# yhn112/DeDLOC

Measured on AMD Instinct MI355X. Metric: samples/sec (whole node) ALBERT-large MLM pretrain at 1/2/4/8 peers, higher is better.
Workload: dtype bf16; 1 GPU; model=albert-large-v2, global_batch=4096, seq_len=512, parallelism=collaborative-dp1, micro_batch=512, grad_accum=1, compression=FLOAT16, optimizer=LAMB, impl=dedloc

## Files before the change

dedloc_amd/csrc/include/dl_attn_tile.h:

```cpp
#pragma once

#include "dl_common.h"

namespace {

typedef __bf16 bf16x8 __attribute__((ext_vector_type(8)));
typedef short s4_t __attribute__((ext_vector_type(4)));
typedef short s8_t __attribute__((ext_vector_type(8)));
typedef __attribute__((address_space(3))) s4_t lds_s4;

constexpr int TILE_BYTES = 64 * 128;
constexpr float NEG_BIG = -1.0e30f;

__device__ __forceinline__ int swzf(int x) { return x ^ ((x & 1) << 2); }
__device__ __forceinline__ int chunk_off(int row, int c) { return row * 128 + ((c ^ swzf((row >> 1) & 7)) << 4); }
__device__ __forceinline__ int crow(int i, int hh) { return (i & 3) + 8 * (i >> 2) + 4 * hh; }

__device__ __forceinline__ floatx16 mfma32(bf16x8 a, bf16x8 b, floatx16 c) {
  return __builtin_amdgcn_mfma_f32_32x32x16_bf16(a, b, c, 0, 0, 0);
}

__device__ __forceinline__ bf16x8 lds_row_frag(const uint8_t* tile, int row, int c) {
  return *reinterpret_cast<const bf16x8*>(tile + chunk_off(row, c));
}

__device__ __forceinline__ s4_t lds_tr(const uint8_t* tile, int row0, int col0, int i) {
  const int row = row0 + (i >> 2);
  const int col = col0 + 4 * (i & 3);
  const int off = chunk_off(row, col >> 3) + ((col & 7) << 1);
  return __builtin_amdgcn_ds_read_tr16_b64_v4i16((lds_s4*)(tile + off));
}

__device__ __forceinline__ bf16x8 tr_operand(const uint8_t* tile, int kbase, int hh, int t, int lane) {
  const int col0 = 32 * t + 16 * ((lane >> 4) & 1);
  const s4_t lo = lds_tr(tile, kbase + 4 * hh, col0, lane & 15);
  const s4_t hi = lds_tr(tile, kbase + 8 + 4 * hh, col0, lane & 15);
  const s8_t v = __builtin_shufflevector(lo, hi, 0, 1, 2, 3, 4, 5, 6, 7);
  return __builtin_bit_cast(bf16x8, v);
}

__device__ __forceinline__ bf16x8 pack_acc(const floatx16& x, int s) {
  bf16x8 b;
#pragma unroll
  for (int e = 0; e < 8; ++e) b[e] = (__bf16)x[8 * s + e];
  return b;
}

__device__ __forceinline__ bf16x8 gload8(const bf16_t* p) { return *reinterpret_cast<const bf16x8*>(p); }

typedef __attribute__((address_space(3))) void lds_void;

__device__ __forceinline__ uint32_t lds_u32(const void* p) {
  return __builtin_amdgcn_readfirstlane((uint32_t)(size_t)(const lds_void*)p);
}
__device__ __forceinline__ void dma16(const void* g, uint32_t lds) {
  asm volatile("s_mov_b32 m0, %0\n\tglobal_load_lds_dwordx4 %1, off" ::"s"(lds), "v"(g) : "memory", "m0");
}
__device__ __forceinline__ void dma4(const void* g, uint32_t lds) {
  asm volatile("s_mov_b32 m0, %0\n\tglobal_load_lds_dword %1, off" ::"s"(lds), "v"(g) : "memory", "m0");
}

__device__ __forceinline__ void wait_vm_all() {
  asm volatile("" ::: "memory");
  __builtin_amdgcn_s_waitcnt(0x0F70);
}
template <typename T>
__device__ __forceinline__ void settle(T& v) { asm volatile("" : "+v"(v)); }

template <int NW = 4>
__device__ __forceinline__ void dma_tile(const bf16_t* g, long ld, int row0, uint8_t* tile, int w, int lane) {
#pragma unroll
  for (int j = 0; j < 8 / NW; ++j) {
    const int p = w + NW * j;
    const int row = 8 * p + (lane >> 3);
    const int c = (lane & 7) ^ swzf((row >> 1) & 7);
    dma16(g + (long)(row0 + row) * ld + c * 8, lds_u32(tile + p * 1024));
  }
}

__device__ __forceinline__ void dma_f32x64(const float* g, uint8_t* dst, int lane) {
  dma4(g + lane, lds_u32(dst));
}

template <int N>
__device__ __forceinline__ void wait_cnt(int ahead) {
  if (ahead >= 2) asm volatile("s_waitcnt vmcnt(%0)" ::"n"(2 * N) : "memory");
  else if (ahead == 1) asm volatile("s_waitcnt vmcnt(%0)" ::"n"(N) : "memory");
  else asm volatile("s_waitcnt vmcnt(0)" ::: "memory");
}
template <int PIECES = 4>
__device__ __forceinline__ void wait_stages(int ahead, bool bias) {
  if (bias) wait_cnt<PIECES + 1>(ahead);
  else wait_cnt<PIECES>(ahead);
}

__device__ __forceinline__ void store4(bf16_t* p, float a, float b, float c, float d) {
  uint2 v;
  v.x = (uint32_t)f2bf(a) | ((uint32_t)f2bf(b) << 16);
  v.y = (uint32_t)f2bf(c) | ((uint32_t)f2bf(d) << 16);
  *reinterpret_cast<uint2*>(p) = v;
}

constexpr float RESCALE_THR = 8.f;

struct BlockId {
  int x, h, b;
};
__device__ __forceinline__ BlockId block_id(int xcd) {
  const int gx = gridDim.x, gy = gridDim.y;
  const int n = gx * gy * gridDim.z;
  int p = blockIdx.x + gx * (blockIdx.y + gy * blockIdx.z);
  if (xcd && (n & 7) == 0) p = (p & 7) * (n >> 3) + (p >> 3);
  return BlockId{p % gx, (p / gx) % gy, p / (gx * gy)};
}

__device__ __forceinline__ int kv_end_of(const int* kvinfo, int B, int b, int S, bool& use_len) {
  use_len = false;
  if (kvinfo == nullptr || kvinfo[B] == 0) return S;
  const int len = kvinfo[b];
  if (len <= 0 || len > S) return S;
  use_len = true;
  return len;
}

template <bool VARLEN>
__device__ __forceinline__ int seq_rows(const int* info, int b, int S) {
  if constexpr (VARLEN) return info[b + 1] - info[b];
  else return S;
}
template <bool VARLEN>
__device__ __forceinline__ long seq_base(const int* info, int b, int S) {
  if constexpr (VARLEN) return info[b];
  else return (long)b * S;
}
template <bool VARLEN>
__device__ __forceinline__ int seq_kv_end(const int* info, int B, int b, int S, bool& use_len) {
  if constexpr (VARLEN) {
    use_len = true;
    return info[B + 1 + b];
  } else {
    return kv_end_of(info, B, b, S, use_len);
  }
}
template <bool VARLEN>
__device__ __forceinline__ long seq_stat(int b, int h, int H, int S, int T, long rb) {
  if constexpr (VARLEN) return (long)h * T + rb;
  else return ((long)b * H + h) * S;
}

__device__ __forceinline__ float vmax3(float a, float b, float c) {
  float r;
  asm("v_max3_f32 %0, %1, %2, %3" : "=v"(r) : "v"(a), "v"(b), "v"(c));
  return r;
}

__device__ __forceinline__ float half_max(float x) {
  const auto r = __builtin_amdgcn_permlane32_swap(__float_as_uint(x), __float_as_uint(x), false, false);
  float m;
  asm("v_max_f32 %0, %1, %2" : "=v"(m) : "v"(__uint_as_float(r[0])), "v"(__uint_as_float(r[1])));
  return m;
}
__device__ __forceinline__ float half_sum(float x) {
  const auto r = __builtin_amdgcn_permlane32_swap(__float_as_uint(x), __float_as_uint(x), false, false);
  return __uint_as_float(r[0]) + __uint_as_float(r[1]);
}

}
```

dedloc_amd/csrc/kernels/attention.hip:

```cpp
#include <cstdlib>
#include <type_traits>

#include "dl_attn_tile.h"
#include "dl_common.h"
#include "dl_kernels.h"

namespace {

constexpr int HD = 64;

struct TileRegs { uint4 a, b; };

__device__ __forceinline__ uint4 tile_ld1(const bf16_t* g, long ld, int row0, int rows_valid, int idx) {
  const int row = min(row0 + (idx >> 3), rows_valid - 1);
  return *reinterpret_cast<const uint4*>(g + (long)row * ld + (idx & 7) * 8);
}

__device__ __forceinline__ void tile_load(TileRegs& t, const bf16_t* g, long ld, int row0, int rows_valid) {
  t.a = tile_ld1(g, ld, row0, rows_valid, threadIdx.x);
  t.b = tile_ld1(g, ld, row0, rows_valid, threadIdx.x + 256);
}

__device__ __forceinline__ void tile_store(const TileRegs& t, uint8_t* tile) {
  const int i0 = threadIdx.x, i1 = threadIdx.x + 256;
  *reinterpret_cast<uint4*>(tile + chunk_off(i0 >> 3, i0 & 7)) = t.a;
  *reinterpret_cast<uint4*>(tile + chunk_off(i1 >> 3, i1 & 7)) = t.b;
}

constexpr int NBUF = 2;
constexpr int STAGE = 2 * TILE_BYTES + 512;


struct FwdCtx {
  const bf16_t* Kg;
  const bf16_t* Vg;
  long ld;
  int S, kv_end;
  const float* mb_g;
  float sl2;
  uint8_t* smem;
  float* mbs;
  int w, lane;
  template <int NW = 4>
  __device__ __forceinline__ void issue(int s) const {
    uint8_t* slot = smem + (s % NBUF) * STAGE;
    dma_tile<NW>(Kg, ld, s * 64, slot, w, lane);
    dma_tile<NW>(Vg, ld, s * 64, slot + TILE_BYTES, w, lane);
    if (mb_g) dma_f32x64(mb_g + s * 64, slot + 2 * TILE_BYTES, lane);
  }
};

__device__ __forceinline__ float key_bias(const FwdCtx& c, int key) {
  return c.mb_g ? c.mb_g[key] : (key < c.kv_end ? 0.f : NEG_BIG);
}

template <bool LEAN, bool RING, int QS, int NW>
__device__ __forceinline__ void fwd_tiles(const FwdCtx& c, int kt0, int kt1, int nt, const bf16x8 (&qf)[QS][4],
                                          floatx16 (&o)[QS][2], float (&m)[QS], float (&l)[QS], int r, int hh,
                                          int lane) {
  TileRegs kr, vr;
  float mbr = 0.f;
  for (int kt = kt0; kt < kt1; ++kt) {
    const uint8_t* Ks;
    const float* mb;
    bool more = false;
    if constexpr (RING) {
      wait_stages<16 / NW>(min(nt - 1 - kt, NBUF - 2), c.mb_g != nullptr);
      __syncthreads();
      if (kt + NBUF - 1 < nt) c.template issue<NW>(kt + NBUF - 1);
      Ks = c.smem + (kt % NBUF) * STAGE;
      mb = reinterpret_cast<const float*>(Ks + 2 * TILE_BYTES);
    } else {
      const int cur = kt & 1;
      Ks = c.smem + cur * 2 * TILE_BYTES;
      mb = c.mbs + cur * 64;
      more = kt + 1 < nt;
      if (more) {
        tile_load(kr, c.Kg, c.ld, (kt + 1) * 64, c.S);
        tile_load(vr, c.Vg, c.ld, (kt + 1) * 64, c.S);
        if (threadIdx.x < 64) mbr = key_bias(c, (kt + 1) * 64 + threadIdx.x);
      }
    }
    const uint8_t* Vs = Ks + TILE_BYTES;
    floatx16 s[QS][2];
#pragma unroll
    for (int u = 0; u < QS; ++u)
#pragma unroll
      for (int j = 0; j < 2; ++j)
#pragma unroll
        for (int i = 0; i < 16; ++i) s[u][j][i] = 0.f;
#pragma unroll
    for (int j = 0; j < 2; ++j)
#pragma unroll
      for (int ks = 0; ks < 4; ++ks) {
        const bf16x8 kfr = lds_row_frag(Ks, 32 * j + r, 2 * ks + hh);
#pragma unroll
        for (int u = 0; u < QS; ++u) s[u][j] = mfma32(kfr, qf[u][ks], s[u][j]);
      }
#pragma unroll
    for (int u = 0; u < QS; ++u) {
      if (!LEAN) {
        if (!RING || c.mb_g) {
#pragma unroll
          for (int j = 0; j < 2; ++j)
#pragma unroll
            for (int i = 0; i < 16; ++i) s[u][j][i] = fmaf(s[u][j][i], c.sl2, mb[32 * j + crow(i, hh)]);
        } else {
#pragma unroll
          for (int j = 0; j < 2; ++j)
#pragma unroll
            for (int i = 0; i < 16; ++i)
              s[u][j][i] = fmaf(s[u][j][i], c.sl2, kt * 64 + 32 * j + crow(i, hh) < c.kv_end ? 0.f : NEG_BIG);
        }
      }
      float mc[4];
#pragma unroll
      for (int q4 = 0; q4 < 4; ++q4) {
        const floatx16& sv = s[u][q4 >> 1];
        const int o8 = (q4 & 1) * 8;
        float v = vmax3(sv[o8], sv[o8 + 1], sv[o8 + 2]);
        v = vmax3(v, sv[o8 + 3], sv[o8 + 4]);
        v = vmax3(v, sv[o8 + 5], sv[o8 + 6]);
        mc[q4] = v;
      }
      float mx = vmax3(vmax3(mc[0], mc[1], s[u][0][7]), vmax3(mc[2], mc[3], s[u][0][15]),
                       vmax3(s[u][1][7], s[u][1][15], mc[0]));
      mx = half_max(mx);
      if (LEAN) mx *= c.sl2;
      const bool grow = mx > m[u] + RESCALE_THR;
      if (__ballot(grow) != 0) {
        const float mn = grow ? mx : m[u];
        const float alpha = __builtin_amdgcn_exp2f(m[u] - mn);
        l[u] *= alpha;
        m[u] = mn;
#pragma unroll
        for (int t = 0; t < 2; ++t)
#pragma unroll
          for (int i = 0; i < 16; ++i) o[u][t][i] *= alpha;
      }
      const float nm = -m[u];
      float rsa[8] = {0.f, 0.f, 0.f, 0.f, 0.f, 0.f, 0.f, 0.f};
#pragma unroll
      for (int j = 0; j < 2; ++j)
#pragma unroll
        for (int i = 0; i < 16; ++i) {
          const float pv = __builtin_amdgcn_exp2f(LEAN ? fmaf(s[u][j][i], c.sl2, nm) : s[u][j][i] + nm);
          s[u][j][i] = pv;
          rsa[i & 7] += pv;
        }
      float rs = ((rsa[0] + rsa[1]) + (rsa[2] + rsa[3])) + ((rsa[4] + rsa[5]) + (rsa[6] + rsa[7]));
      l[u] += half_sum(rs);
    }
#pragma unroll
    for (int j = 0; j < 2; ++j)
#pragma unroll
      for (int ss = 0; ss < 2; ++ss) {
        bf16x8 pb[QS];
#pragma unroll
        for (int u = 0; u < QS; ++u) pb[u] = pack_acc(s[u][j], ss);
#pragma unroll
        for (int t = 0; t < 2; ++t) {
          const bf16x8 vfr = tr_operand(Vs, 32 * j + 16 * ss, hh, t, lane);
#pragma unroll
          for (int u = 0; u < QS; ++u) o[u][t] = mfma32(vfr, pb[u], o[u][t]);
        }
      }
    if constexpr (!RING) {
      if (more) {
        uint8_t* Kn = c.smem + ((kt & 1) ^ 1) * 2 * TILE_BYTES;
        tile_store(kr, Kn);
        tile_store(vr, Kn + TILE_BYTES);
        if (threadIdx.x < 64) c.mbs[((kt & 1) ^ 1) * 64 + threadIdx.x] = mbr;
      }
      __syncthreads();
    }
  }
}

template <bool RING, int QS, int NW = 4, bool VARLEN = false>
__global__ __launch_bounds__(64 * NW, NW == 8 ? 1 : 2) void attn_fwd_kernel(const bf16_t* __restrict__ qkv, long ld,
                                                          const float* __restrict__ mbias,
                                                          const int* __restrict__ kvinfo, bf16_t* __restrict__ out,
                                                          long ldo, float* __restrict__ lse, int B, int H, int S_,
                                                          float sl2, int xcd) {
  __shared__ __attribute__((aligned(16))) uint8_t smem[RING ? NBUF * STAGE : 4 * TILE_BYTES + 2 * 64 * 4];
  const BlockId bid = block_id(xcd);
  const int b = bid.b, h = bid.h;
  const int lane = threadIdx.x & 63, w = threadIdx.x >> 6, r = lane & 31, hh = lane >> 5;
  const int S = seq_rows<VARLEN>(kvinfo, b, S_);
  if constexpr (VARLEN) {
    if (bid.x * (32 * QS * NW) >= S) return;
  }
  const long rb = seq_base<VARLEN>(kvinfo, b, S);
  const bf16_t* Qg = qkv + rb * ld + h * HD;
  bool use_len;
  FwdCtx c;
  c.Kg = qkv + rb * ld + (long)H * HD + h * HD;
  c.Vg = qkv + rb * ld + 2L * H * HD + h * HD;
  c.ld = ld;
  c.S = S;
  c.kv_end = seq_kv_end<VARLEN>(kvinfo, B, b, S, use_len);
  c.mb_g = (!use_len && mbias) ? mbias + rb : nullptr;
  c.sl2 = sl2;
  c.smem = smem;
  c.mbs = reinterpret_cast<float*>(smem + 4 * TILE_BYTES);
  c.w = w;
  c.lane = lane;

  static_assert(NW == 4 || (NW == 8 && RING), "8-wave blocks stage through the ring");
  const int nt = (c.kv_end + 63) / 64;
  if constexpr (RING) {
    for (int s0 = 0; s0 < NBUF - 1 && s0 < nt; ++s0) c.template issue<NW>(s0);
  }
  int q[QS];
  bf16x8 qf[QS][4];
#pragma unroll
  for (int u = 0; u < QS; ++u) {
    q[u] = bid.x * (32 * QS * NW) + w * (32 * QS) + 32 * u + r;
    const int qc = min(q[u], S - 1);
#pragma unroll
    for (int ks = 0; ks < 4; ++ks) qf[u][ks] = gload8(Qg + (long)qc * ld + ks * 16 + 8 * hh);
    if constexpr (RING) {
#pragma unroll
      for (int ks = 0; ks < 4; ++ks) settle(qf[u][ks]);
    }
  }

  floatx16 o[QS][2];
  float m[QS], l[QS];
#pragma unroll
  for (int u = 0; u < QS; ++u) {
    m[u] = NEG_BIG;
    l[u] = 0.f;
#pragma unroll
    for (int t = 0; t < 2; ++t)
#pragma unroll
      for (int i = 0; i < 16; ++i) o[u][t][i] = 0.f;
  }

  if constexpr (RING) {
    wait_vm_all();
  } else {
    TileRegs kr, vr;
    tile_load(kr, c.Kg, ld, 0, S);
    tile_load(vr, c.Vg, ld, 0, S);
    const float mbr = threadIdx.x < 64 ? key_bias(c, threadIdx.x) : 0.f;
    tile_store(kr, smem);
    tile_store(vr, smem + TILE_BYTES);
    if (threadIdx.x < 64) c.mbs[threadIdx.x] = mbr;
    __syncthreads();
  }
  const int nlean = c.mb_g ? 0 : c.kv_end / 64;
  fwd_tiles<true, RING, QS, NW>(c, 0, nlean, nt, qf, o, m, l, r, hh, lane);
  fwd_tiles<false, RING, QS, NW>(c, nlean, nt, nt, qf, o, m, l, r, hh, lane);

#pragma unroll
  for (int u = 0; u < QS; ++u) {
    if (q[u] < S) {
      const float inv = 1.f / l[u];
      bf16_t* op = out + (rb + q[u]) * ldo + h * HD;
#pragma unroll
      for (int t = 0; t < 2; ++t)
#pragma unroll
        for (int v = 0; v < 4; ++v)
          store4(op + 32 * t + 8 * v + 4 * hh, o[u][t][4 * v] * inv, o[u][t][4 * v + 1] * inv,
                 o[u][t][4 * v + 2] * inv, o[u][t][4 * v + 3] * inv);
      if (hh == 0) lse[seq_stat<VARLEN>(b, h, H, S, S_, rb) + q[u]] = m[u] + log2f(l[u]);
    }
  }
}

template <bool RING, int QS, bool VARLEN = false>
__global__ __launch_bounds__(256, 2) void attn_bwd_dq_kernel(const bf16_t* __restrict__ qkv, long ld,
                                                             const float* __restrict__ mbias,
                                                             const int* __restrict__ kvinfo,
                                                             const bf16_t* __restrict__ out, const bf16_t* __restrict__ dout,
                                                             long ldo, const float* __restrict__ lse,
                                                             float* __restrict__ delta, bf16_t* __restrict__ dqkv,
                                                             float* __restrict__ dbias, int B, int H, int S_, float sl2,
                                                             float scale, int xcd) {
  __shared__ __attribute__((aligned(16))) uint8_t smem[RING ? NBUF * STAGE : 4 * TILE_BYTES + 4 * 64 * 4];
  const BlockId bid = block_id(xcd);
  const int b = bid.b, h = bid.h;
  const int lane = threadIdx.x & 63, w = threadIdx.x >> 6, r = lane & 31, hh = lane >> 5;
  const int S = seq_rows<VARLEN>(kvinfo, b, S_);
  if constexpr (VARLEN) {
    if (bid.x * (128 * QS) >= S) return;
  }
  const long rb = seq_base<VARLEN>(kvinfo, b, S);
  const bf16_t* Qg = qkv + rb * ld + h * HD;
  const bf16_t* Kg = qkv + rb * ld + (long)H * HD + h * HD;
  const bf16_t* Vg = qkv + rb * ld + 2L * H * HD + h * HD;
  bool use_len;
  const int kv_end = seq_kv_end<VARLEN>(kvinfo, B, b, S, use_len);
  const float* mb_g = (!use_len && mbias) ? mbias + rb : nullptr;
  float* mbs = reinterpret_cast<float*>(smem + 4 * TILE_BYTES);
  const int nt = (kv_end + 63) / 64;
  auto issue = [&](int st) {
    uint8_t* slot = smem + (st % NBUF) * STAGE;
    dma_tile(Kg, ld, st * 64, slot, w, lane);
    dma_tile(Vg, ld, st * 64, slot + TILE_BYTES, w, lane);
    if (mb_g) dma_f32x64(mb_g + st * 64, slot + 2 * TILE_BYTES, lane);
  };
  if constexpr (RING) {
    for (int s0 = 0; s0 < NBUF - 1 && s0 < nt; ++s0) issue(s0);
  }

  int q[QS];
  bf16x8 qf[QS][4], df[QS][4];
  float dl[QS], l2[QS];
#pragma unroll
  for (int u = 0; u < QS; ++u) {
    q[u] = bid.x * (128 * QS) + w * (32 * QS) + 32 * u + r;
    const int qc = min(q[u], S - 1);
    dl[u] = 0.f;
#pragma unroll
    for (int ks = 0; ks < 4; ++ks) {
      qf[u][ks] = gload8(Qg + (long)qc * ld + ks * 16 + 8 * hh);
      const long oo = (rb + qc) * ldo + h * HD + ks * 16 + 8 * hh;
      df[u][ks] = gload8(dout + oo);
      const bf16x8 of = gload8(out + oo);
#pragma unroll
      for (int e = 0; e < 8; ++e) dl[u] += (float)df[u][ks][e] * (float)of[e];
    }
    dl[u] += __shfl_xor(dl[u], 32, 64);
    l2[u] = lse[seq_stat<VARLEN>(b, h, H, S, S_, rb) + qc];
    if constexpr (RING) {
      settle(l2[u]);
      settle(dl[u]);
#pragma unroll
      for (int ks = 0; ks < 4; ++ks) {
        settle(qf[u][ks]);
        settle(df[u][ks]);
      }
    }
  }

  floatx16 dq[QS][2];
#pragma unroll
  for (int u = 0; u < QS; ++u)
#pragma unroll
    for (int t = 0; t < 2; ++t)
#pragma unroll
      for (int i = 0; i < 16; ++i) dq[u][t][i] = 0.f;

  TileRegs kr, vr;
  float mbr = 0.f;
  if constexpr (RING) {
    wait_vm_all();
  } else {
    tile_load(kr, Kg, ld, 0, S);
    tile_load(vr, Vg, ld, 0, S);
    if (threadIdx.x < 64) mbr = mb_g ? mb_g[threadIdx.x] : 0.f;
    tile_store(kr, smem);
    tile_store(vr, smem + TILE_BYTES);
    if (threadIdx.x < 64) mbs[threadIdx.x] = mbr;
    __syncthreads();
  }

  for (int kt = 0; kt < nt; ++kt) {
    const uint8_t* Ks;
    const float* mb;
    if constexpr (RING) {
      wait_stages(min(nt - 1 - kt, NBUF - 2), mb_g != nullptr);
      __syncthreads();
      if (kt + NBUF - 1 < nt) issue(kt + NBUF - 1);
      Ks = smem + (kt % NBUF) * STAGE;
      mb = reinterpret_cast<const float*>(Ks + 2 * TILE_BYTES);
    } else {
      Ks = smem + (kt & 1) * 2 * TILE_BYTES;
      mb = mbs + (kt & 1) * 64;
      if (kt + 1 < nt) {
        tile_load(kr, Kg, ld, (kt + 1) * 64, S);
        tile_load(vr, Vg, ld, (kt + 1) * 64, S);
        if (threadIdx.x < 64) mbr = mb_g ? mb_g[(kt + 1) * 64 + threadIdx.x] : 0.f;
      }
    }
    const uint8_t* Vs = Ks + TILE_BYTES;
    const bool interior = mb_g == nullptr && (kt + 1) * 64 <= kv_end;
#pragma unroll
    for (int j = 0; j < 2; ++j) {
      floatx16 st[QS], dp[QS];
#pragma unroll
      for (int u = 0; u < QS; ++u)
#pragma unroll
        for (int i = 0; i < 16; ++i) { st[u][i] = 0.f; dp[u][i] = 0.f; }
#pragma unroll
      for (int ks = 0; ks < 4; ++ks) {
        const bf16x8 kfr = lds_row_frag(Ks, 32 * j + r, 2 * ks + hh);
        const bf16x8 vfr = lds_row_frag(Vs, 32 * j + r, 2 * ks + hh);
#pragma unroll
        for (int u = 0; u < QS; ++u) {
          st[u] = mfma32(kfr, qf[u][ks], st[u]);
          dp[u] = mfma32(vfr, df[u][ks], dp[u]);
        }
      }
#pragma unroll
      for (int u = 0; u < QS; ++u) {
        if (interior) {
#pragma unroll
          for (int i = 0; i < 16; ++i) {
            const float p = __builtin_amdgcn_exp2f(fmaf(st[u][i], sl2, -l2[u]));
            st[u][i] = p * (dp[u][i] - dl[u]);
          }
        } else {
#pragma unroll
          for (int i = 0; i < 16; ++i) {
            const int key = kt * 64 + 32 * j + crow(i, hh);
            const float bias = mb_g ? mb[32 * j + crow(i, hh)] : (key < kv_end ? 0.f : NEG_BIG);
            const float p = __builtin_amdgcn_exp2f(st[u][i] * sl2 + bias - l2[u]);
            st[u][i] = p * (dp[u][i] - dl[u]);
          }
        }
      }
#pragma unroll
      for (int ss = 0; ss < 2; ++ss) {
        bf16x8 pb[QS];
#pragma unroll
        for (int u = 0; u < QS; ++u) pb[u] = pack_acc(st[u], ss);
#pragma unroll
        for (int t = 0; t < 2; ++t) {
          const bf16x8 ktr = tr_operand(Ks, 32 * j + 16 * ss, hh, t, lane);
#pragma unroll
          for (int u = 0; u < QS; ++u) dq[u][t] = mfma32(ktr, pb[u], dq[u][t]);
        }
      }
    }
    if constexpr (!RING) {
      if (kt + 1 < nt) {
        uint8_t* Kn = smem + ((kt & 1) ^ 1) * 2 * TILE_BYTES;
        tile_store(kr, Kn);
        tile_store(vr, Kn + TILE_BYTES);
        if (threadIdx.x < 64) mbs[((kt & 1) ^ 1) * 64 + threadIdx.x] = mbr;
      }
      __syncthreads();
    }
  }
  if constexpr (RING) __syncthreads();
#pragma unroll
  for (int u = 0; u < QS; ++u) {
    if (q[u] < S && hh == 0) delta[seq_stat<VARLEN>(b, h, H, S, S_, rb) + q[u]] = dl[u];
    if (q[u] < S) {
      bf16_t* dp_ = dqkv + (rb + q[u]) * ld + h * HD;
#pragma unroll
      for (int t = 0; t < 2; ++t)
#pragma unroll
        for (int v = 0; v < 4; ++v)
          store4(dp_ + 32 * t + 8 * v + 4 * hh, dq[u][t][4 * v] * scale, dq[u][t][4 * v + 1] * scale,
                 dq[u][t][4 * v + 2] * scale, dq[u][t][4 * v + 3] * scale);
    }
  }
  if (dbias) {
    float* red = reinterpret_cast<float*>(smem);
    float* part = red + 4 * 32 * 64;
    auto chunk_addr = [&](int row, int ch) { return red + (w * 32 + row) * 64 + ((ch ^ (row & 15)) << 2); };
#pragma unroll
    for (int u = 0; u < QS; ++u) {
      const bool live = q[u] < S;
#pragma unroll
      for (int which = 0; which < 2; ++which) {
        if (which == 0) {
#pragma unroll
          for (int t = 0; t < 2; ++t)
#pragma unroll
            for (int v4 = 0; v4 < 4; ++v4) {
              float4 v = float4{0.f, 0.f, 0.f, 0.f};
              if (live)
                v = float4{round_bf16(dq[u][t][4 * v4] * scale), round_bf16(dq[u][t][4 * v4 + 1] * scale),
                           round_bf16(dq[u][t][4 * v4 + 2] * scale), round_bf16(dq[u][t][4 * v4 + 3] * scale)};
              *reinterpret_cast<float4*>(chunk_addr(r, 8 * t + 2 * v4 + hh)) = v;
            }
        } else {
#pragma unroll
          for (int ks = 0; ks < 4; ++ks)
#pragma unroll
            for (int g = 0; g < 2; ++g) {
              float4 v = float4{0.f, 0.f, 0.f, 0.f};
              if (live)
                v = float4{(float)df[u][ks][4 * g], (float)df[u][ks][4 * g + 1], (float)df[u][ks][4 * g + 2],
                           (float)df[u][ks][4 * g + 3]};
              *reinterpret_cast<float4*>(chunk_addr(r, 4 * ks + 2 * hh + g)) = v;
            }
        }
        __syncthreads();
        {
          const int c = lane;
          float sum = 0.f;
#pragma unroll 8
          for (int row = 0; row < 32; ++row)
            sum += red[(w * 32 + row) * 64 + (((c >> 2) ^ (row & 15)) << 2) + (c & 3)];
          part[w * 64 + c] = sum;
        }
        __syncthreads();
        if (threadIdx.x < 64) {
          const int c = threadIdx.x;
          atomicAdd(&dbias[(which ? 2L * H * HD : 0L) + h * HD + c],
                    part[c] + part[64 + c] + part[128 + c] + part[192 + c]);
        }
        __syncthreads();
      }
    }
  }
}

template <bool RING, int KS, bool VARLEN = false>
__global__ __launch_bounds__(256, KS == 2 ? 1 : 2) void attn_bwd_dkdv_kernel(
    const bf16_t* __restrict__ qkv, long ld, const float* __restrict__ mbias, const int* __restrict__ kvinfo,
    const bf16_t* __restrict__ dout, long ldo, const float* __restrict__ lse, const float* __restrict__ delta,
    bf16_t* __restrict__ dqkv, int B, int H, int S_, float sl2, float scale, int xcd) {
  __shared__ __attribute__((aligned(16))) uint8_t smem[RING ? NBUF * STAGE : 4 * TILE_BYTES + 2 * 2 * 64 * 4];
  const BlockId bid = block_id(xcd);
  const int b = bid.b, h = bid.h;
  const int lane = threadIdx.x & 63, w = threadIdx.x >> 6, r = lane & 31, hh = lane >> 5;
  const int S = seq_rows<VARLEN>(kvinfo, b, S_);
  if constexpr (VARLEN) {
    if (bid.x * (128 * KS) >= S) return;
  }
  const long rb = seq_base<VARLEN>(kvinfo, b, S);
  const bf16_t* Qg = qkv + rb * ld + h * HD;
  const bf16_t* Kg = qkv + rb * ld + (long)H * HD + h * HD;
  const bf16_t* Vg = qkv + rb * ld + 2L * H * HD + h * HD;
  const bf16_t* dOg = dout + rb * ldo + h * HD;
  const float* lse_g = lse + seq_stat<VARLEN>(b, h, H, S, S_, rb);
  const float* del_g = delta + seq_stat<VARLEN>(b, h, H, S, S_, rb);
  float* rowv = reinterpret_cast<float*>(smem + 4 * TILE_BYTES);

  int k[KS];
#pragma unroll
  for (int u = 0; u < KS; ++u) k[u] = bid.x * (128 * KS) + w * (32 * KS) + 32 * u + r;
  bool use_len;
  const int kv_end = seq_kv_end<VARLEN>(kvinfo, B, b, S, use_len);
  if (use_len && bid.x * (128 * KS) >= kv_end) {
#pragma unroll
    for (int u = 0; u < KS; ++u) {
      if (k[u] < S) {
        bf16_t* dkp = dqkv + (rb + k[u]) * ld + (long)H * HD + h * HD;
        bf16_t* dvp = dqkv + (rb + k[u]) * ld + 2L * H * HD + h * HD;
#pragma unroll
        for (int v = 0; v < 8; ++v) {
          store4(dkp + 8 * v + 4 * hh, 0.f, 0.f, 0.f, 0.f);
          store4(dvp + 8 * v + 4 * hh, 0.f, 0.f, 0.f, 0.f);
        }
      }
    }
    return;
  }
  const int nt = S / 64;
  auto issue = [&](int st) {
    uint8_t* slot = smem + (st % NBUF) * STAGE;
    dma_tile(Qg, ld, st * 64, slot, w, lane);
    dma_tile(dOg, ldo, st * 64, slot + TILE_BYTES, w, lane);
    dma_f32x64((w < 2 ? lse_g : del_g) + st * 64, slot + 2 * TILE_BYTES + (w < 2 ? 0 : 256), lane);
  };
  if constexpr (RING) {
    for (int s0 = 0; s0 < NBUF - 1 && s0 < nt; ++s0) issue(s0);
  }
  bf16x8 kf[KS][4], vf[KS][4];
  float mbk[KS];
#pragma unroll
  for (int u = 0; u < KS; ++u) {
    const int kc = min(k[u], S - 1);
#pragma unroll
    for (int ks = 0; ks < 4; ++ks) {
      kf[u][ks] = gload8(Kg + (long)kc * ld + ks * 16 + 8 * hh);
      vf[u][ks] = gload8(Vg + (long)kc * ld + ks * 16 + 8 * hh);
    }
    mbk[u] = use_len ? (k[u] < kv_end ? 0.f : NEG_BIG) : (mbias ? mbias[rb + kc] : 0.f);
    if constexpr (RING) {
      settle(mbk[u]);
#pragma unroll
      for (int ks = 0; ks < 4; ++ks) {
        settle(kf[u][ks]);
        settle(vf[u][ks]);
      }
    }
  }

  floatx16 dk[KS][2], dv[KS][2];
#pragma unroll
  for (int u = 0; u < KS; ++u)
#pragma unroll
    for (int t = 0; t < 2; ++t)
#pragma unroll
      for (int i = 0; i < 16; ++i) { dk[u][t][i] = 0.f; dv[u][t][i] = 0.f; }

  TileRegs qr, dr;
  float rv = 0.f;
  if constexpr (RING) {
    wait_vm_all();
  } else {
    tile_load(qr, Qg, ld, 0, S);
    tile_load(dr, dOg, ldo, 0, S);
    if (threadIdx.x < 128) rv = threadIdx.x < 64 ? lse_g[threadIdx.x] : del_g[threadIdx.x - 64];
    tile_store(qr, smem);
    tile_store(dr, smem + TILE_BYTES);
    if (threadIdx.x < 128) rowv[threadIdx.x] = rv;
    __syncthreads();
  }

  auto qloop = [&](auto lean_tag) {
  constexpr bool LEAN = decltype(lean_tag)::value;
  for (int qt = 0; qt < nt; ++qt) {
    const uint8_t* Qs;
    const float* lse_s;
    if constexpr (RING) {
      wait_stages(min(nt - 1 - qt, NBUF - 2), true);
      __syncthreads();
      if (qt + NBUF - 1 < nt) issue(qt + NBUF - 1);
      Qs = smem + (qt % NBUF) * STAGE;
      lse_s = reinterpret_cast<const float*>(Qs + 2 * TILE_BYTES);
    } else {
      Qs = smem + (qt & 1) * 2 * TILE_BYTES;
      lse_s = rowv + (qt & 1) * 128;
      if (qt + 1 < nt) {
        tile_load(qr, Qg, ld, (qt + 1) * 64, S);
        tile_load(dr, dOg, ldo, (qt + 1) * 64, S);
        if (threadIdx.x < 128)
          rv = threadIdx.x < 64 ? lse_g[(qt + 1) * 64 + threadIdx.x] : del_g[(qt + 1) * 64 + threadIdx.x - 64];
      }
    }
    const uint8_t* Ds = Qs + TILE_BYTES;
    const float* del_s = lse_s + 64;
#pragma unroll
    for (int i2 = 0; i2 < 2; ++i2) {
      floatx16 sc[KS], dp[KS];
#pragma unroll
      for (int u = 0; u < KS; ++u)
#pragma unroll
        for (int i = 0; i < 16; ++i) { sc[u][i] = 0.f; dp[u][i] = 0.f; }
#pragma unroll
      for (int ks = 0; ks < 4; ++ks) {
        const bf16x8 qfr = lds_row_frag(Qs, 32 * i2 + r, 2 * ks + hh);
        const bf16x8 dfr = lds_row_frag(Ds, 32 * i2 + r, 2 * ks + hh);
#pragma unroll
        for (int u = 0; u < KS; ++u) {
          sc[u] = mfma32(qfr, kf[u][ks], sc[u]);
          dp[u] = mfma32(dfr, vf[u][ks], dp[u]);
        }
      }
#pragma unroll
      for (int u = 0; u < KS; ++u)
#pragma unroll
        for (int i = 0; i < 16; ++i) {
          const int qq = 32 * i2 + crow(i, hh);
          const float p = __builtin_amdgcn_exp2f(LEAN ? fmaf(sc[u][i], sl2, -lse_s[qq])
                                                      : sc[u][i] * sl2 + mbk[u] - lse_s[qq]);
          sc[u][i] = p;
          dp[u][i] = p * (dp[u][i] - del_s[qq]);
        }
#pragma unroll
      for (int ss = 0; ss < 2; ++ss) {
        bf16x8 pb[KS], db[KS];
#pragma unroll
        for (int u = 0; u < KS; ++u) {
          pb[u] = pack_acc(sc[u], ss);
          db[u] = pack_acc(dp[u], ss);
        }
#pragma unroll
        for (int t = 0; t < 2; ++t) {
          const bf16x8 dtr = tr_operand(Ds, 32 * i2 + 16 * ss, hh, t, lane);
          const bf16x8 qtr = tr_operand(Qs, 32 * i2 + 16 * ss, hh, t, lane);
#pragma unroll
          for (int u = 0; u < KS; ++u) {
            dv[u][t] = mfma32(dtr, pb[u], dv[u][t]);
            dk[u][t] = mfma32(qtr, db[u], dk[u][t]);
          }
        }
      }
    }
    if constexpr (!RING) {
      if (qt + 1 < nt) {
        uint8_t* Qn = smem + ((qt & 1) ^ 1) * 2 * TILE_BYTES;
        tile_store(qr, Qn);
        tile_store(dr, Qn + TILE_BYTES);
        if (threadIdx.x < 128) rowv[((qt & 1) ^ 1) * 128 + threadIdx.x] = rv;
      }
      __syncthreads();
    }
  }
  };
  if (use_len) {
    qloop(std::true_type{});
#pragma unroll
    for (int u = 0; u < KS; ++u)
      if (k[u] >= kv_end)
#pragma unroll
        for (int t = 0; t < 2; ++t)
#pragma unroll
          for (int i = 0; i < 16; ++i) dk[u][t][i] = dv[u][t][i] = 0.f;
  } else {
    qloop(std::false_type{});
  }
#pragma unroll
  for (int u = 0; u < KS; ++u) {
    if (k[u] < S) {
      bf16_t* dkp = dqkv + (rb + k[u]) * ld + (long)H * HD + h * HD;
      bf16_t* dvp = dqkv + (rb + k[u]) * ld + 2L * H * HD + h * HD;
#pragma unroll
      for (int t = 0; t < 2; ++t)
#pragma unroll
        for (int v = 0; v < 4; ++v) {
          store4(dkp + 32 * t + 8 * v + 4 * hh, dk[u][t][4 * v] * scale, dk[u][t][4 * v + 1] * scale,
                 dk[u][t][4 * v + 2] * scale, dk[u][t][4 * v + 3] * scale);
          store4(dvp + 32 * t + 8 * v + 4 * hh, dv[u][t][4 * v], dv[u][t][4 * v + 1], dv[u][t][4 * v + 2],
                 dv[u][t][4 * v + 3]);
        }
    }
  }
}

constexpr int kAttnXcd = 1;

}

int dl_attn_fwd(const bf16_t* qkv, long ld, const float* mbias, const int* kvinfo, bf16_t* out, long ldo, float* lse,
                int B, int H, int S, int D, float scale, hipStream_t st) {
  if (D == 128) return dl_attn_hd128_fwd(qkv, ld, mbias, kvinfo, out, ldo, lse, B, H, S, scale, st);
  if (D != HD || S % 64 != 0 || ld % 8 != 0 || ldo % 8 != 0) return -1;
  const float sl2 = scale * 1.4426950408889634f;
  dim3 grid((S + 255) / 256, H, B);
  attn_fwd_kernel<true, 2><<<grid, 256, 0, st>>>(qkv, ld, mbias, kvinfo, out, ldo, lse, B, H, S, sl2, kAttnXcd);
  return 0;
}

int dl_attn_bwd(const bf16_t* qkv, long ld, const float* mbias, const int* kvinfo, const bf16_t* out,
                const bf16_t* dout, long ldo, const float* lse, float* delta, bf16_t* dqkv, float* dbias, int B, int H,
                int S, int D, float scale, hipStream_t st) {
  if (D == 128)
    return dl_attn_hd128_bwd(qkv, ld, mbias, kvinfo, out, dout, ldo, lse, delta, dqkv, dbias, B, H, S, scale, st);
  if (D != HD || S % 64 != 0 || ld % 8 != 0 || ldo % 8 != 0) return -1;
  const float sl2 = scale * 1.4426950408889634f;
  dim3 grid_dq((S + 255) / 256, H, B);
  attn_bwd_dq_kernel<true, 2><<<grid_dq, 256, 0, st>>>(qkv, ld, mbias, kvinfo, out, dout, ldo, lse, delta, dqkv,
                                                       dbias, B, H, S, sl2, scale, kAttnXcd);
  dim3 grid_kv((S + 127) / 128, H, B);
  attn_bwd_dkdv_kernel<false, 1><<<grid_kv, 256, 0, st>>>(qkv, ld, mbias, kvinfo, dout, ldo, lse, delta, dqkv, B, H,
                                                          S, sl2, scale, kAttnXcd);
  return 0;
}

int dl_attn_varlen_fwd(const bf16_t* qkv, long ld, const int* seqinfo, bf16_t* out, long ldo, float* lse, int B, int T,
                       int max_slot, int H, int D, float scale, hipStream_t st) {
  if (!seqinfo || B < 1 || T % 64 != 0 || max_slot < 64 || max_slot % 64 != 0 || max_slot > T) return -1;
  if (D == 128) return dl_attn_hd128_varlen_fwd(qkv, ld, seqinfo, out, ldo, lse, B, T, max_slot, H, scale, st);
  if (D != HD || ld % 8 != 0 || ldo % 8 != 0) return -1;
  const float sl2 = scale * 1.4426950408889634f;
  dim3 grid((max_slot + 255) / 256, H, B);
  attn_fwd_kernel<true, 2, 4, true><<<grid, 256, 0, st>>>(qkv, ld, nullptr, seqinfo, out, ldo, lse, B, H, T, sl2,
                                                          kAttnXcd);
  return 0;
}

int dl_attn_varlen_bwd(const bf16_t* qkv, long ld, const int* seqinfo, const bf16_t* out, const bf16_t* dout, long ldo,
                       const float* lse, float* delta, bf16_t* dqkv, float* dbias, int B, int T, int max_slot, int H,
                       int D, float scale, hipStream_t st) {
  if (!seqinfo || B < 1 || T % 64 != 0 || max_slot < 64 || max_slot % 64 != 0 || max_slot > T) return -1;
  if (D == 128)
    return dl_attn_hd128_varlen_bwd(qkv, ld, seqinfo, out, dout, ldo, lse, delta, dqkv, dbias, B, T, max_slot, H, scale,
                                    st);
  if (D != HD || ld % 8 != 0 || ldo % 8 != 0) return -1;
  const float sl2 = scale * 1.4426950408889634f;
  dim3 grid_dq((max_slot + 255) / 256, H, B);
  attn_bwd_dq_kernel<true, 2, true><<<grid_dq, 256, 0, st>>>(qkv, ld, nullptr, seqinfo, out, dout, ldo, lse, delta,
                                                             dqkv, dbias, B, H, T, sl2, scale, kAttnXcd);
  dim3 grid_kv((max_slot + 127) / 128, H, B);
  attn_bwd_dkdv_kernel<false, 1, true><<<grid_kv, 256, 0, st>>>(qkv, ld, nullptr, seqinfo, dout, ldo, lse, delta, dqkv,
                                                                B, H, T, sl2, scale, kAttnXcd);
  return 0;
}
```

Baseline: 984.0 samples/s.

## Split attention backward into lean/masked tile loops and widen output stores

The dQ backward loop is split into a lean phase with no masking for full interior key tiles and a masked phase, with bias and length masks now separate branches. Output rows for O, dQ, dK and dV are written as 16-byte stores after a permlane32 swap instead of 8-byte stores. The dbias reduction moves from an LDS transpose with several barriers to DPP/permlane half-wave sums plus a single barrier. The dK/dV kernel's first template argument changes from false to true (apparently enabling the ring/DMA path), which alters its load pipelining. The aim is to cut per-tile branching, store instructions and sync overhead in attention backward, at the cost of more complex code and possible register pressure.

```diff
diff --git a/dedloc_amd/csrc/include/dl_attn_tile.h b/dedloc_amd/csrc/include/dl_attn_tile.h
--- a/dedloc_amd/csrc/include/dl_attn_tile.h
+++ b/dedloc_amd/csrc/include/dl_attn_tile.h
@@ -101,6 +101,36 @@
   *reinterpret_cast<uint2*>(p) = v;
 }
 
+__device__ __forceinline__ uint2 pack4(float a, float b, float c, float d) {
+  uint2 v;
+  v.x = (uint32_t)f2bf(a) | ((uint32_t)f2bf(b) << 16);
+  v.y = (uint32_t)f2bf(c) | ((uint32_t)f2bf(d) << 16);
+  return v;
+}
+
+__device__ __forceinline__ void store_row64(bf16_t* row, const floatx16 (&x)[2], float scale, int hh, bool live) {
+#pragma unroll
+  for (int t = 0; t < 2; ++t)
+#pragma unroll
+    for (int vp = 0; vp < 2; ++vp) {
+      const int i0 = 8 * vp;
+      uint2 a = pack4(x[t][i0] * scale, x[t][i0 + 1] * scale, x[t][i0 + 2] * scale, x[t][i0 + 3] * scale);
+      uint2 b = pack4(x[t][i0 + 4] * scale, x[t][i0 + 5] * scale, x[t][i0 + 6] * scale, x[t][i0 + 7] * scale);
+      const auto rx = __builtin_amdgcn_permlane32_swap(a.x, b.x, false, false);
+      const auto ry = __builtin_amdgcn_permlane32_swap(a.y, b.y, false, false);
+      if (live) *reinterpret_cast<uint4*>(row + 32 * t + 16 * vp + 8 * hh) = make_uint4(rx[0], ry[0], rx[1], ry[1]);
+    }
+}
+
+__device__ __forceinline__ float half_wave_sum(float v) {
+  v += dpp_f32<0xB1>(v);
+  v += dpp_f32<0x4E>(v);
+  v += dpp_f32<0x141>(v);
+  v += dpp_f32<0x140>(v);
+  const auto r = __builtin_amdgcn_permlane16_swap(__float_as_uint(v), __float_as_uint(v), false, false);
+  return __uint_as_float(r[0]) + __uint_as_float(r[1]);
+}
+
 constexpr float RESCALE_THR = 8.f;
 
 struct BlockId {
diff --git a/dedloc_amd/csrc/kernels/attention.hip b/dedloc_amd/csrc/kernels/attention.hip
--- a/dedloc_amd/csrc/kernels/attention.hip
+++ b/dedloc_amd/csrc/kernels/attention.hip
@@ -256,17 +256,9 @@
 
 #pragma unroll
   for (int u = 0; u < QS; ++u) {
-    if (q[u] < S) {
-      const float inv = 1.f / l[u];
-      bf16_t* op = out + (rb + q[u]) * ldo + h * HD;
-#pragma unroll
-      for (int t = 0; t < 2; ++t)
-#pragma unroll
-        for (int v = 0; v < 4; ++v)
-          store4(op + 32 * t + 8 * v + 4 * hh, o[u][t][4 * v] * inv, o[u][t][4 * v + 1] * inv,
-                 o[u][t][4 * v + 2] * inv, o[u][t][4 * v + 3] * inv);
-      if (hh == 0) lse[seq_stat<VARLEN>(b, h, H, S, S_, rb) + q[u]] = m[u] + log2f(l[u]);
-    }
+    const bool live = q[u] < S;
+    store_row64(out + (rb + q[u]) * ldo + h * HD, o[u], 1.f / l[u], hh, live);
+    if (live && hh == 0) lse[seq_stat<VARLEN>(b, h, H, S, S_, rb) + q[u]] = m[u] + log2f(l[u]);
   }
 }
 
@@ -358,7 +350,12 @@
     __syncthreads();
   }
 
-  for (int kt = 0; kt < nt; ++kt) {
+  auto tiles = [&](auto lean_tag, int kt0, int kt1) {
+  constexpr bool LEAN = decltype(lean_tag)::value;
+  int tm = threadIdx.x;
+  if constexpr (!LEAN) settle(tm);
+  const int lm = tm & 63, rm = tm & 31, hm = (tm >> 5) & 1;
+  for (int kt = kt0; kt < kt1; ++kt) {
     const uint8_t* Ks;
     const float* mb;
     if constexpr (RING) {
@@ -377,7 +374,6 @@
       }
     }
     const uint8_t* Vs = Ks + TILE_BYTES;
-    const bool interior = mb_g == nullptr && (kt + 1) * 64 <= kv_end;
 #pragma unroll
     for (int j = 0; j < 2; ++j) {
       floatx16 st[QS], dp[QS];
@@ -387,8 +383,8 @@
         for (int i = 0; i < 16; ++i) { st[u][i] = 0.f; dp[u][i] = 0.f; }
 #pragma unroll
       for (int ks = 0; ks < 4; ++ks) {
-        const bf16x8 kfr = lds_row_frag(Ks, 32 * j + r, 2 * ks + hh);
-        const bf16x8 vfr = lds_row_frag(Vs, 32 * j + r, 2 * ks + hh);
+        const bf16x8 kfr = lds_row_frag(Ks, 32 * j + rm, 2 * ks + hm);
+        const bf16x8 vfr = lds_row_frag(Vs, 32 * j + rm, 2 * ks + hm);
 #pragma unroll
         for (int u = 0; u < QS; ++u) {
           st[u] = mfma32(kfr, qf[u][ks], st[u]);
@@ -397,20 +393,25 @@
       }
 #pragma unroll
       for (int u = 0; u < QS; ++u) {
-        if (interior) {
+        if constexpr (LEAN) {
 #pragma unroll
           for (int i = 0; i < 16; ++i) {
             const float p = __builtin_amdgcn_exp2f(fmaf(st[u][i], sl2, -l2[u]));
             st[u][i] = p * (dp[u][i] - dl[u]);
           }
-        } else {
+        } else if (mb_g) {
 #pragma unroll
           for (int i = 0; i < 16; ++i) {
-            const int key = kt * 64 + 32 * j + crow(i, hh);
-            const float bias = mb_g ? mb[32 * j + crow(i, hh)] : (key < kv_end ? 0.f : NEG_BIG);
-            const float p = __builtin_amdgcn_exp2f(st[u][i] * sl2 + bias - l2[u]);
+            const float p = __builtin_amdgcn_exp2f(st[u][i] * sl2 + mb[32 * j + crow(i, hm)] - l2[u]);
             st[u][i] = p * (dp[u][i] - dl[u]);
           }
+        } else {
+#pragma unroll
+          for (int i = 0; i < 16; ++i) {
+            const int key = kt * 64 + 32 * j + crow(i, hm);
+            const float p = __builtin_amdgcn_exp2f(st[u][i] * sl2 + (key < kv_end ? 0.f : NEG_BIG) - l2[u]);
+            st[u][i] = p * (dp[u][i] - dl[u]);
+          }
         }
       }
 #pragma unroll
@@ -420,7 +421,7 @@
         for (int u = 0; u < QS; ++u) pb[u] = pack_acc(st[u], ss);
 #pragma unroll
         for (int t = 0; t < 2; ++t) {
-          const bf16x8 ktr = tr_operand(Ks, 32 * j + 16 * ss, hh, t, lane);
+          const bf16x8 ktr = tr_operand(Ks, 32 * j + 16 * ss, hm, t, lm);
 #pragma unroll
           for (int u = 0; u < QS; ++u) dq[u][t] = mfma32(ktr, pb[u], dq[u][t]);
         }
@@ -436,69 +437,64 @@
       __syncthreads();
     }
   }
+  };
+  const int nlean = mb_g ? 0 : kv_end / 64;
+  tiles(std::true_type{}, 0, nlean);
+  tiles(std::false_type{}, nlean, nt);
   if constexpr (RING) __syncthreads();
+  int tid = threadIdx.x;
+  settle(tid);
+  const int w_ = tid >> 6, r_ = tid & 31, hh_ = (tid >> 5) & 1;
+  int qe[QS];
+#pragma unroll
+  for (int u = 0; u < QS; ++u) qe[u] = bid.x * (128 * QS) + w_ * (32 * QS) + 32 * u + r_;
 #pragma unroll
   for (int u = 0; u < QS; ++u) {
-    if (q[u] < S && hh == 0) delta[seq_stat<VARLEN>(b, h, H, S, S_, rb) + q[u]] = dl[u];
-    if (q[u] < S) {
-      bf16_t* dp_ = dqkv + (rb + q[u]) * ld + h * HD;
+    const bool live = qe[u] < S;
+    if (live && hh_ == 0) delta[seq_stat<VARLEN>(b, h, H, S, S_, rb) + qe[u]] = dl[u];
+    store_row64(dqkv + (rb + qe[u]) * ld + h * HD, dq[u], scale, hh_, live);
+  }
+  if (dbias) {
+    float* part = reinterpret_cast<float*>(smem);
+    float cq[2][16], cd[4][8];
+#pragma unroll
+    for (int t = 0; t < 2; ++t)
+#pragma unroll
+      for (int i = 0; i < 16; ++i) {
+        float v = 0.f;
+#pragma unroll
+        for (int u = 0; u < QS; ++u) v += qe[u] < S ? round_bf16(dq[u][t][i] * scale) : 0.f;
+        cq[t][i] = half_wave_sum(v);
+      }
+#pragma unroll
+    for (int ks = 0; ks < 4; ++ks)
+#pragma unroll
+      for (int e = 0; e < 8; ++e) {
+        float v = 0.f;
+#pragma unroll
+        for (int u = 0; u < QS; ++u) v += qe[u] < S ? (float)df[u][ks][e] : 0.f;
+        cd[ks][e] = half_wave_sum(v);
+      }
+    if (r_ == 0) {
+      float* pw = part + w_ * 128;
 #pragma unroll
       for (int t = 0; t < 2; ++t)
 #pragma unroll
-        for (int v = 0; v < 4; ++v)
-          store4(dp_ + 32 * t + 8 * v + 4 * hh, dq[u][t][4 * v] * scale, dq[u][t][4 * v + 1] * scale,
-                 dq[u][t][4 * v + 2] * scale, dq[u][t][4 * v + 3] * scale);
-    }
-  }
-  if (dbias) {
-    float* red = reinterpret_cast<float*>(smem);
-    float* part = red + 4 * 32 * 64;
-    auto chunk_addr = [&](int row, int ch) { return red + (w * 32 + row) * 64 + ((ch ^ (row & 15)) << 2); };
-#pragma unroll
-    for (int u = 0; u < QS; ++u) {
-      const bool live = q[u] < S;
-#pragma unroll
-      for (int which = 0; which < 2; ++which) {
-        if (which == 0) {
-#pragma unroll
-          for (int t = 0; t < 2; ++t)
-#pragma unroll
-            for (int v4 = 0; v4 < 4; ++v4) {
-              float4 v = float4{0.f, 0.f, 0.f, 0.f};
-              if (live)
-                v = float4{round_bf16(dq[u][t][4 * v4] * scale), round_bf16(dq[u][t][4 * v4 + 1] * scale),
-                           round_bf16(dq[u][t][4 * v4 + 2] * scale), round_bf16(dq[u][t][4 * v4 + 3] * scale)};
-              *reinterpret_cast<float4*>(chunk_addr(r, 8 * t + 2 * v4 + hh)) = v;
-            }
-        } else {
-#pragma unroll
-          for (int ks = 0; ks < 4; ++ks)
-#pragma unroll
-            for (int g = 0; g < 2; ++g) {
-              float4 v = float4{0.f, 0.f, 0.f, 0.f};
-              if (live)
-                v = float4{(float)df[u][ks][4 * g], (float)df[u][ks][4 * g + 1], (float)df[u][ks][4 * g + 2],
-                           (float)df[u][ks][4 * g + 3]};
-              *reinterpret_cast<float4*>(chunk_addr(r, 4 * ks + 2 * hh + g)) = v;
-            }
-        }
-        __syncthreads();
-        {
-          const int c = lane;
-          float sum = 0.f;
-#pragma unroll 8
-          for (int row = 0; row < 32; ++row)
-            sum += red[(w * 32 + row) * 64 + (((c >> 2) ^ (row & 15)) << 2) + (c & 3)];
-          part[w * 64 + c] = sum;
-        }
-        __syncthreads();
-        if (threadIdx.x < 64) {
-          const int c = threadIdx.x;
-          atomicAdd(&dbias[(which ? 2L * H * HD : 0L) + h * HD + c],
-                    part[c] + part[64 + c] + part[128 + c] + part[192 + c]);
-        }
-        __syncthreads();
-      }
+        for (int v4 = 0; v4 < 4; ++v4)
+          *reinterpret_cast<float4*>(pw + 32 * t + 8 * v4 + 4 * hh_) =
+              float4{cq[t][4 * v4], cq[t][4 * v4 + 1], cq[t][4 * v4 + 2], cq[t][4 * v4 + 3]};
+#pragma unroll
+      for (int ks = 0; ks < 4; ++ks)
+#pragma unroll
+        for (int g = 0; g < 2; ++g)
+          *reinterpret_cast<float4*>(pw + 64 + 16 * ks + 8 * hh_ + 4 * g) =
+              float4{cd[ks][4 * g], cd[ks][4 * g + 1], cd[ks][4 * g + 2], cd[ks][4 * g + 3]};
+    }
+    __syncthreads();
+    if (threadIdx.x < 128) {
+      const int c = threadIdx.x & 63, which = threadIdx.x >> 6;
+      const float* pc = part + which * 64 + c;
+      atomicAdd(&dbias[(which ? 2L * H * HD : 0L) + h * HD + c], pc[0] + pc[128] + pc[256] + pc[384]);
     }
   }
 }
@@ -693,19 +689,9 @@
   }
 #pragma unroll
   for (int u = 0; u < KS; ++u) {
-    if (k[u] < S) {
-      bf16_t* dkp = dqkv + (rb + k[u]) * ld + (long)H * HD + h * HD;
-      bf16_t* dvp = dqkv + (rb + k[u]) * ld + 2L * H * HD + h * HD;
-#pragma unroll
-      for (int t = 0; t < 2; ++t)
-#pragma unroll
-        for (int v = 0; v < 4; ++v) {
-          store4(dkp + 32 * t + 8 * v + 4 * hh, dk[u][t][4 * v] * scale, dk[u][t][4 * v + 1] * scale,
-                 dk[u][t][4 * v + 2] * scale, dk[u][t][4 * v + 3] * scale);
-          store4(dvp + 32 * t + 8 * v + 4 * hh, dv[u][t][4 * v], dv[u][t][4 * v + 1], dv[u][t][4 * v + 2],
-                 dv[u][t][4 * v + 3]);
-        }
-    }
+    const bool live = k[u] < S;
+    store_row64(dqkv + (rb + k[u]) * ld + (long)H * HD + h * HD, dk[u], scale, hh, live);
+    store_row64(dqkv + (rb + k[u]) * ld + 2L * H * HD + h * HD, dv[u], 1.f, hh, live);
   }
 }
 
@@ -734,8 +720,8 @@
   attn_bwd_dq_kernel<true, 2><<<grid_dq, 256, 0, st>>>(qkv, ld, mbias, kvinfo, out, dout, ldo, lse, delta, dqkv,
                                                        dbias, B, H, S, sl2, scale, kAttnXcd);
   dim3 grid_kv((S + 127) / 128, H, B);
-  attn_bwd_dkdv_kernel<false, 1><<<grid_kv, 256, 0, st>>>(qkv, ld, mbias, kvinfo, dout, ldo, lse, delta, dqkv, B, H,
-                                                          S, sl2, scale, kAttnXcd);
+  attn_bwd_dkdv_kernel<true, 1><<<grid_kv, 256, 0, st>>>(qkv, ld, mbias, kvinfo, dout, ldo, lse, delta, dqkv, B, H,
+                                                         S, sl2, scale, kAttnXcd);
   return 0;
 }
 
@@ -764,7 +750,7 @@
   attn_bwd_dq_kernel<true, 2, true><<<grid_dq, 256, 0, st>>>(qkv, ld, nullptr, seqinfo, out, dout, ldo, lse, delta,
                                                              dqkv, dbias, B, H, T, sl2, scale, kAttnXcd);
   dim3 grid_kv((max_slot + 127) / 128, H, B);
-  attn_bwd_dkdv_kernel<false, 1, true><<<grid_kv, 256, 0, st>>>(qkv, ld, nullptr, seqinfo, dout, ldo, lse, delta, dqkv,
-                                                                B, H, T, sl2, scale, kAttnXcd);
+  attn_bwd_dkdv_kernel<true, 1, true><<<grid_kv, 256, 0, st>>>(qkv, ld, nullptr, seqinfo, dout, ldo, lse, delta, dqkv,
+                                                               B, H, T, sl2, scale, kAttnXcd);
   return 0;
 }
```

Measured after the change: 996.0 samples/s, median of 6. 1.2% higher.
